# bobocode/lmono

Measured on AMD Instinct MI355X. Metric: KITTI HDL-64 scans/sec (scanRegistration + laserOdometry), higher is better.
Workload: dtype f32 features / f64 solve

## Files before the change

lmono_amd/csrc/batch.hpp:

```cpp
#pragma once
#include "common.hpp"

namespace lmono {

constexpr int kCornerTable = 16384;
constexpr int kSurfTable = 131072;
constexpr unsigned long long kEmptyKey = ~0ull;

struct __attribute__((aligned(16))) GridCell {
    unsigned long long key;
    int start;
    int cnt;
};

struct BatchView {
    const float4 *in;
    const int64_t *off;
    int n_scans;
    int scan0;
    int n_lines;
    int n_limit;
    int has_grid;
    float min_range;
    float4 *cloud;
    float *curv;
    int8_t *label;
    uint8_t *gap;
    int8_t *ring_tmp;
    int *seg_hist;
    int *scan_ends;
    int *scan_half;
    float *scan_ori;
    int *ring_begin;
    int *n_cloud;
    int *status;
    int *sel_sharp;
    int *sel_sharp_n;
    int *sel_flat;
    int *sel_flat_n;
    float4 *lf_tmp;
    int *lf_n;
    int *sel_todo;
    int *li_todo;
    int *vox_todo;
    float4 *sharp;
    float4 *less_sharp;
    float4 *flat;
    float4 *less_flat;
    int *feat_n;
    int *line_first_ge;
    int *line_last_le;
    GridCell *cg_cell;
    GridCell *sg_cell;
    float4 *cg_pts;
    float4 *sg_pts;
    float4 *lbc_pts;
    float4 *lbs_pts;
    int *lb_start;
    float4 *lb_elev;
    int *grid_mask;
};

}
```

lmono_amd/csrc/frontend.hip:

```cpp
#include "batch.hpp"

namespace lmono {

__device__ __forceinline__ int ring_of(float angle, int n_lines, bool &discard)
{
    int id = 0;
    discard = false;
    if (n_lines == 16) {
        id = (int)((double)((angle + 15.0f) / 2.0f) + 0.5);
        if (id > n_lines - 1 || id < 0) discard = true;
    } else if (n_lines == 32) {
        id = (int)(((double)angle + 92.0 / 3.0) * 3.0 / 4.0);
        if (id > n_lines - 1 || id < 0) discard = true;
    } else {
        if ((double)angle >= -8.83)
            id = (int)((double)(2.0f - angle) * 3.0 + 0.5);
        else
            id = n_lines / 2 + (int)((-8.83 - (double)angle) * 2.0 + 0.5);
        if ((double)angle > 2.0 || (double)angle < -24.33 || id > 50 || id < 0) discard = true;
    }
    return id;
}

__device__ __forceinline__ bool point_valid(const float4 &p, float mr2)
// ... 873 lines not shown
        for (int w = 0; w < wave; w++) base += scr[48 + w];
        n_out = scr[48] + scr[49] + scr[50] + scr[51];
        int o = base;
        for (int t = t_lo; t < t_hi; t++) {
            const unsigned int c = (unsigned int)(keys[t] >> 32);
            if (t == 0 || c != (unsigned int)(keys[t - 1] >> 32)) {
                float sx = 0.f, sy = 0.f, sz = 0.f, si = 0.f;
                int cnt = 0;
                for (int u = t; u < nseg && (unsigned int)(keys[u] >> 32) == c; u++) {
                    const int i0 = (int)(keys[u] & 0xffffffffull);
                    int rl = 1;
                    while (i0 + rl < len && ((contw[(i0 + rl) >> 6] >> ((i0 + rl) & 63)) & 1ull)) rl++;
                    for (int b4 = 0; b4 < rl; b4 += 4) {
                        float4 q4[4];
#pragma unroll
                        for (int k = 0; k < 4; k++) q4[k] = b4 + k < rl ? cl[i0 + b4 + k] : make_float4(0.f, 0.f, 0.f, 0.f);
#pragma unroll
                        for (int k = 0; k < 4; k++) if (b4 + k < rl) { sx += q4[k].x; sy += q4[k].y; sz += q4[k].z; si += q4[k].w; }
                    }
                    cnt += rl;
                }
                const float fc = (float)cnt;
                outp[o++] = make_float4(sx / fc, sy / fc, sz / fc, si / fc);
            }
        }
    }
    VT(6)
#ifdef LMONO_VOX_PROF
    if (blockIdx.x == 20 && blockIdx.y == 3 && tid == 0) printf("VOX len %d nseg %d nout %d | load %lld bbox+cell %lld heads %lld sort %lld runs %lld accum %lld\n", len, nseg, n_out, vt[1]-vt[0], vt[2]-vt[1], vt[3]-vt[2], vt[4]-vt[3], vt[5]-vt[4], vt[6]-vt[5]);
#endif
    if (tid == 0) b.lf_n[s * 64 + r] = n_out;
}

#ifndef LMONO_COMPACT_T
#define LMONO_COMPACT_T 256
#endif
constexpr int kCompT = LMONO_COMPACT_T;
static_assert(kCompT >= 256 && kCompT % 64 == 0, "the four prefixes take one wave each");

template <int kT>
__device__ __forceinline__ void compact_scan(const BatchView &b, int s, int &n_ls_out, int &n_lf_out)
{
    const int tid = threadIdx.x;
    const int64_t off = b.off[s];
    constexpr int NE = kMaxRings * kSectors;
    __shared__ int pre_sh[NE + 1], pre_ls[NE + 1], pre_fl[NE + 1], pre_lf[kMaxRings + 1];
    const int *nsh = b.sel_sharp_n + s * NE;
    const int *nfl = b.sel_flat_n + s * NE;
    {
        const int lane = tid & 63, wave = tid >> 6;
        constexpr int kPer = NE / 64;
        int c[kPer], sum = 0;
        if (wave < 4) {
        const int *srcp = wave <= 1 ? nsh : (wave == 2 ? nfl : b.lf_n + s * 64);
#pragma unroll
        for (int q = 0; q < kPer; q++) {
            const int e = lane * kPer + q;
            const bool on = wave < 3 || e < kMaxRings;
            c[q] = srcp[on ? e : 0];
            if (!on) c[q] = 0;
        }
#pragma unroll
        for (int q = 0; q < kPer; q++) {
            if (wave == 0) c[q] = min(c[q], 2);
            sum += c[q];
        }
        const int incl = wave_scan_incl(sum);
        int run = incl - sum;
        int *dst = wave == 0 ? pre_sh : (wave == 1 ? pre_ls : (wave == 2 ? pre_fl : pre_lf));
        const int n_e = wave == 3 ? kMaxRings : NE;
#pragma unroll
        for (int q = 0; q < kPer; q++) {
// ... 74 lines not shown
        for (int q = 0; q < 4; q++) {
            const int j = j0 + kT * q;
            if (j < n_lf) {
                lf[j] = v4[q];
                int v = (int)v4[q].w;
                v = v < 0 ? 0 : (v > 65 ? 65 : v);
                atomicMin(&s_first[1][v], j);
                atomicMax(&s_last[1][v], j);
            }
        }
    }
    if (tid == 0) {
        b.feat_n[s * 4 + 0] = pre_sh[NE]; b.feat_n[s * 4 + 1] = pre_ls[NE];
        b.feat_n[s * 4 + 2] = pre_fl[NE]; b.feat_n[s * 4 + 3] = n_lf;
    }
    __syncthreads();
    for (int x = tid; x < 2 * 66 * 66; x += kT) {
        const int cld = x / (66 * 66), y = x % (66 * 66), a = y / 66, bb = y % 66;
        if (a >= bb + 3 && s_first[cld][a] < s_last[cld][bb]) s_flag[cld] = 1;
    }
    __syncthreads();
    if (tid == 0 || tid == 64) {
        const int cld = tid >> 6;
        const int n = cld ? n_lf : pre_ls[NE];
        int *first_ge = b.line_first_ge + (size_t)(s * 2 + cld) * 66, *last_le = b.line_last_le + (size_t)(s * 2 + cld) * 66;
        int m = n;
        for (int t = 65; t >= 0; t--) { m = min(m, s_first[cld][t] == INT_MAX ? n : s_first[cld][t]); first_ge[t] = m; }
        int M = -1;
        for (int t = 0; t <= 65; t++) { M = max(M, s_last[cld][t]); last_le[t] = M; }
        if (s_flag[cld]) atomicOr(b.status + s, kStatusIrregularLines);
    }
    n_ls_out = pre_ls[NE]; n_lf_out = n_lf;
}

__global__ __launch_bounds__(kCompT) void k_compact(BatchView b)
{
    int n_ls, n_lf;
    compact_scan<kCompT>(b, b.scan0 + blockIdx.x, n_ls, n_lf);
}

}
```

lmono_amd/csrc/lmono_hip.hip:

```cpp
#include "frontend.hip"
#include "odometry.hip"
#include "corr_flat.hip"
#include "mapping.hip"
#include "ba.hip"
#include "ba_solve.hip"
#include "feat.hip"
#include "marg.hip"

#include <string>
#include <vector>
#include <thread>
#include <mutex>
#include <condition_variable>
#include <atomic>
#include <functional>
#include <memory>
#include <chrono>
#include <algorithm>
#include <cstdio>
#include <cstring>

constexpr int kListGrid = 256;

using namespace lmono;
// ... 95 lines not shown
#ifdef LMONO_DIAG_SEARCH
extern "C" const char *lmono_version(void) { return "lmono-hip 0.4 (gfx950, diagnostic build: + hash-grid search)"; }
#else
extern "C" const char *lmono_version(void) { return "lmono-hip 0.4 (gfx950)"; }
#endif

extern "C" lmono_ctx *lmono_create(int device)
{
    int n = 0;
    if (hipGetDeviceCount(&n) != hipSuccess || n <= 0 || device < 0 || device >= n) return nullptr;
    if (hipSetDevice(device) != hipSuccess) return nullptr;
    lmono_ctx *c = new lmono_ctx();
    c->device = device;
    if (const char *e = getenv("LMONO_ODOM_STREAM_PRIORITY")) c->odom_prio = atoi(e) != 0;
    if (const char *e = getenv("GPU_MAX_HW_QUEUES")) c->many_queues = atoi(e) >= 8;
    {
        hipDeviceProp_t prop;
        if (hipGetDeviceProperties(&prop, device) != hipSuccess) { delete c; return nullptr; }
        c->n_cu = prop.multiProcessorCount;
        int per_cu = 0;
        if (hipOccupancyMaxActiveBlocksPerMultiprocessor(&per_cu, (const void *)k_ba_solve<true, false>, kBaT, 0) != hipSuccess || per_cu < 1) per_cu = 1;
        c->cluster_budget = std::max(8, c->n_cu * per_cu / 2);
        c->map_budget = std::max(8, c->n_cu / 2);
        if (const char *e = getenv("LMONO_CLUSTER_BUDGET")) { const int v = atoi(e); if (v >= 1) c->cluster_budget = c->map_budget = v; }
    }
    if (hipMalloc((void **)&c->stats_d, 320) != hipSuccess || hipMemset(c->stats_d, 0, 320) != hipSuccess) { delete c; return nullptr; }
    if (hipFuncSetAttribute((const void *)k_select, hipFuncAttributeMaxDynamicSharedMemorySize, 4 * sel_slice_bytes(kRingCap) + 4 * kSelScratch) != hipSuccess) { delete c; return nullptr; }
    if (hipFuncSetAttribute((const void *)k_voxel<kVoxSmallSlots, kVoxSmallBits, true>, hipFuncAttributeMaxDynamicSharedMemorySize, kVoxLdsSmall) != hipSuccess) { delete c; return nullptr; }
    if (hipFuncSetAttribute((const void *)k_voxel<kVoxBigSlots, kVoxBigBits, false>, hipFuncAttributeMaxDynamicSharedMemorySize, kVoxLdsBig) != hipSuccess) { delete c; return nullptr; }
    if (hipFuncSetAttribute((const void *)k_lm_solve, hipFuncAttributeMaxDynamicSharedMemorySize, kLmRecLds) != hipSuccess) { delete c; return nullptr; }
#ifdef LMONO_DIAG_SEARCH
    if (hipFuncSetAttribute((const void *)k_grid_build, hipFuncAttributeMaxDynamicSharedMemorySize, kGridLds) != hipSuccess) { delete c; return nullptr; }
#endif
    if (hipFuncSetAttribute((const void *)k_line_index<true>, hipFuncAttributeMaxDynamicSharedMemorySize, kLiLdsHalf) != hipSuccess) { delete c; return nullptr; }
    if (hipFuncSetAttribute((const void *)k_compact_index, hipFuncAttributeMaxDynamicSharedMemorySize, kLiLdsHalf) != hipSuccess) { delete c; return nullptr; }
    if (hipFuncSetAttribute((const void *)k_line_index<false>, hipFuncAttributeMaxDynamicSharedMemorySize, kLiLdsFull) != hipSuccess) { delete c; return nullptr; }
    if (hipFuncSetAttribute((const void *)k_marginalize, hipFuncAttributeMaxDynamicSharedMemorySize, (int)sizeof(MargLds)) != hipSuccess) { delete c; return nullptr; }
    if (hipFuncSetAttribute((const void *)k_marg_second_new, hipFuncAttributeMaxDynamicSharedMemorySize, (int)sizeof(Marg2Lds)) != hipSuccess) { delete c; return nullptr; }
#ifdef LMONO_TILE_PROF
    {
        int nb = 0;
        (void)hipOccupancyMaxActiveBlocksPerMultiprocessor(&nb, (const void *)k_corr_flat, kCfT, 0);
        std::fprintf(stderr, "[lmono diag] k_corr_flat: %d workgroups of %d threads per CU by the occupancy query, static LDS %zu B\n", nb, kCfT, sizeof(CfLds));
    }
#endif
    return c;
}

extern "C" void lmono_destroy(lmono_ctx *c)
{
    if (!c) return;
#ifdef LMONO_BOUNDS
    {
        unsigned long long o[4] = { 0, 0, 0, 0 };
        (void)hipDeviceSynchronize();
        if (hipMemcpyFromSymbol(o, HIP_SYMBOL(g_ba_oob), sizeof(o)) == hipSuccess)
            fprintf(stderr, "[lmono bounds] k_ba_solve: %llu access(es) outside the batch's allocation (first: ba_solve.hip:%llu, byte offset %lld, block %llu)\n", o[0], o[1], (long long)o[2], o[3]);
    }
#endif
    for (auto &s : c->sets) { for (auto &e : s.e) (void)hipEventDestroy(e); for (auto &e : s.kev) (void)hipEventDestroy(e); }
    if (c->stats_d) (void)hipFree(c->stats_d);
    for (auto &s : c->gstream) if (s) (void)hipStreamDestroy(s);
    if (c->copy_stream) (void)hipStreamDestroy(c->copy_stream);
    for (void *h : c->stage_all) (void)hipHostFree(h);
    if (c->own_stream) (void)hipStreamDestroy(c->own_stream);
    for (auto &ch : c->arena) (void)hipFree(ch.base);
    for (auto &e : c->gev) if (e) (void)hipEventDestroy(e);
    delete c;
}
// ... 56 lines not shown
    void *q = nullptr;
    if (hipMalloc(&q, (count > 0 ? count : 1) * sizeof(T)) != hipSuccess) return false;
    b->allocs.push_back(q);
    p = (T *)q;
    return true;
}

extern "C" void lmono_batch_destroy(lmono_scan_batch *b)
{
    if (!b) return;
    for (void *p : b->allocs) (void)hipFree(p);
    for (auto &e : b->rep_ev) if (e) (void)hipEventDestroy(e);
    if (b->staged_ev) (void)hipEventDestroy(b->staged_ev);
    if (b->in_free_ev) (void)hipEventDestroy(b->in_free_ev);
    delete b;
}

extern "C" lmono_scan_batch *lmono_batch_create(lmono_ctx *c, int n_cap, int64_t pts_cap)
{
    if (!c || n_cap <= 0 || pts_cap <= 0) return nullptr;
    if (hipSetDevice(c->device) != hipSuccess) return nullptr;
    lmono_scan_batch *b = new lmono_scan_batch();
    b->ctx = c; b->n_cap = n_cap; b->pts_cap = pts_cap;
    BatchView &v = b->v;
    const size_t T = (size_t)pts_cap, N = (size_t)n_cap;
    bool ok = true;
    ok = ok && dalloc(b, b->off_d, N + 1);
    ok = ok && dalloc(b, v.cloud, T) && dalloc(b, v.curv, T) && dalloc(b, v.label, T) && dalloc(b, v.gap, T);
    ok = ok && dalloc(b, v.ring_tmp, T);
    ok = ok && dalloc(b, v.seg_hist, ((T >> 10) + N + 1) * 64) && dalloc(b, v.scan_ends, N * 2) && dalloc(b, v.scan_half, N) && dalloc(b, v.scan_ori, N * 2);
    ok = ok && dalloc(b, v.ring_begin, N * 65) && dalloc(b, v.n_cloud, N) && dalloc(b, v.status, N);
    ok = ok && dalloc(b, v.sel_sharp, N * 64 * 6 * 20) && dalloc(b, v.sel_sharp_n, N * 64 * 6);
    ok = ok && dalloc(b, v.sel_flat, N * 64 * 6 * 4) && dalloc(b, v.sel_flat_n, N * 64 * 6);
    ok = ok && dalloc(b, v.lf_tmp, T) && dalloc(b, v.lf_n, N * 64) && dalloc(b, v.vox_todo, N * 64 + 1) && dalloc(b, v.sel_todo, N * 64 + 1) && dalloc(b, v.li_todo, N * 2 + 1);
    ok = ok && dalloc(b, v.sharp, N * kMaxSharp) && dalloc(b, v.less_sharp, N * kMaxLessSharp);
    ok = ok && dalloc(b, v.flat, N * kMaxFlat) && dalloc(b, v.less_flat, T);
    ok = ok && dalloc(b, v.feat_n, N * 4) && dalloc(b, v.line_first_ge, N * 2 * 66) && dalloc(b, v.line_last_le, N * 2 * 66);
    ok = ok && dalloc(b, v.cg_cell, N * kCornerTable) && dalloc(b, v.sg_cell, N * kSurfTable);
    ok = ok && dalloc(b, v.cg_pts, N * kMaxLessSharp) && dalloc(b, v.sg_pts, T) && dalloc(b, v.grid_mask, N * 2);
    ok = ok && dalloc(b, v.lbc_pts, N * kMaxLessSharp + kLbPad) && dalloc(b, v.lbs_pts, T + kLbPad) && dalloc(b, v.lb_start, N * 2 * (kLineKeys + 1)) && dalloc(b, v.lb_elev, N * 2 * 66);
    ok = ok && dalloc(b, b->incr, N * 7) && dalloc(b, b->poses, N * 7) && dalloc(b, b->xq, 8);
    ok = ok && dalloc(b, b->corr_pair, (size_t)kMaxQueries * 4) && dalloc(b, b->crec_pair, (size_t)kMaxQueries * 4);
    if (!ok) {
        c->err = "lmono_batch_create: hipMalloc failed";
        lmono_batch_destroy(b);
        return nullptr;
    }
    v.off = b->off_d;
    return b;
}

static int rings_used(int n_lines) { return n_lines == 64 ? 51 : n_lines; }

static int check_launch(lmono_ctx *c, const char *what)
{
    hipError_t e = hipGetLastError();
    if (e != hipSuccess) { c->err = std::string(what) + ": " + hipGetErrorString(e); return LMONO_ENODEV; }
    return LMONO_OK;
}

static int scanreg_launch(lmono_ctx *c, lmono_scan_batch *b, int scan0, int n_scans, int64_t max_pts, int n_limit = 0)
{
    BatchView v = b->v;
    v.scan0 = scan0; v.n_limit = n_limit;
    hipStream_t st = c->stream;
    c->ev = c->next_set();
    if (!c->ev) { c->err = "hipEventCreate failed"; return LMONO_ENODEV; }
    c->sets[c->n_sets - 1].reg = true;
    HIP_TRY(c, hipMemsetAsync(v.status + scan0, 0, sizeof(int) * n_scans, st));
    HIP_TRY(c, hipMemsetAsync(v.vox_todo, 0, sizeof(int), st));
    HIP_TRY(c, hipMemsetAsync(v.sel_todo, 0, sizeof(int), st));
    HIP_TRY(c, hipMemsetAsync(v.li_todo, 0, sizeof(int), st));
    HIP_TRY(c, hipEventRecord(c->ev[0], st));
    const int rt_tiles = (int)((max_pts + kRtTile - 1) / kRtTile);
    hipLaunchKernelGGL(k_ring_ends, dim3(n_scans), dim3(256), 0, st, v);
    if (rt_tiles > 0) hipLaunchKernelGGL(k_ring_tag, dim3(rt_tiles, n_scans), dim3(kRtT), 0, st, v);
    hipLaunchKernelGGL(k_ring_offsets, dim3(n_scans), dim3(64), 0, st, v);
    if (rt_tiles > 0) hipLaunchKernelGGL(k_ring_scatter, dim3(rt_tiles, n_scans), dim3(kRtT), 0, st, v);
    HIP_TRY(c, hipEventRecord(c->ev[1], st));
    const int tiles = (int)((max_pts + kCurvTile - 1) / kCurvTile);
#if !LMONO_FUSE_CURV_SELECT
    if (tiles > 0) hipLaunchKernelGGL(k_curvature, dim3(tiles, n_scans), dim3(256), 0, st, v);
#else
    (void)tiles;
#endif
    HIP_TRY(c, hipEventRecord(c->ev[2], st));
    const int n_rings = rings_used(b->v.n_lines);
    HIP_TRY(c, hipMemsetAsync(v.sel_sharp_n + (size_t)scan0 * 64 * 6, 0, sizeof(int) * (size_t)n_scans * 64 * 6, st));
    HIP_TRY(c, hipMemsetAsync(v.sel_flat_n + (size_t)scan0 * 64 * 6, 0, sizeof(int) * (size_t)n_scans * 64 * 6, st));
    HIP_TRY(c, hipMemsetAsync(v.lf_n + (size_t)scan0 * 64, 0, sizeof(int) * (size_t)n_scans * 64, st));
    hipLaunchKernelGGL(k_select, dim3((n_rings + 3) / 4, n_scans), dim3(256), 4 * sel_slice_bytes(kSelSmallCap) + 4 * kSelScratch, st, v, kSelSmallCap, 0);
    hipLaunchKernelGGL(k_select, dim3(kSelBigGrid), dim3(256), 4 * sel_slice_bytes(kRingCap) + 4 * kSelScratch, st, v, (int)kRingCap, 1);
    HIP_TRY(c, hipEventRecord(c->ev[3], st));
    hipLaunchKernelGGL((k_voxel<kVoxSmallSlots, kVoxSmallBits, true>), dim3(n_rings, n_scans), dim3(256), kVoxLdsSmall, st, v);
    hipLaunchKernelGGL((k_voxel<kVoxBigSlots, kVoxBigBits, false>), dim3(kVoxBigGrid), dim3(256), kVoxLdsBig, st, v);
    HIP_TRY(c, hipEventRecord(c->ev[4], st));
#if LMONO_FUSE_COMPACT_INDEX
    hipLaunchKernelGGL(k_compact_index, dim3(n_scans), dim3(kLiT), kLiLdsHalf, st, v);
#else
    hipLaunchKernelGGL(k_compact, dim3(n_scans), dim3(kCompT), 0, st, v);
#endif
    HIP_TRY(c, hipEventRecord(c->ev[5], st));
#ifdef LMONO_DIAG_SEARCH
    if (c->opt[LMONO_OPT_CORR_TILE] != 3) {
        hipLaunchKernelGGL(k_grid_build, dim3(n_scans, 1 + kGridPar), dim3(1024), kGridLds, st, v);
        b->grid_built = true; v.has_grid = 1; b->v.has_grid = 1;
    }
#endif
    HIP_TRY(c, hipEventRecord(c->ev[6], st));
#if !LMONO_FUSE_COMPACT_INDEX
    hipLaunchKernelGGL(k_line_index<true>, dim3(n_scans, 2), dim3(kLiT), kLiLdsHalf, st, v);
#endif
    hipLaunchKernelGGL(k_line_index<false>, dim3(kLiBigGrid), dim3(kLiT), kLiLdsFull, st, v);
    HIP_TRY(c, hipEventRecord(c->ev[7], st));
    return check_launch(c, "scanreg kernels");
}

extern "C" int lmono_scanreg_batch(lmono_ctx *c, lmono_scan_batch *b, const float *xyzi_d, const int64_t *offsets_h,
                                   int n_scans, int n_lines, float min_range);

extern "C" int lmono_scanreg_batch_h(lmono_ctx *c, lmono_scan_batch *b, const float *xyzi_h, const int64_t *offsets_h,
                                     int n_scans, int n_lines, float min_range)
{
    if (!c || !b || !xyzi_h || !offsets_h || n_scans <= 0) return LMONO_EINVAL;
    if (offsets_h[0] != 0) { c->err = "offsets must start at 0"; return LMONO_EINVAL; }
    const int64_t total = offsets_h[n_scans];
    if (total < 0 || total > b->pts_cap) { c->err = "batch: too many points"; return LMONO_ECAPACITY; }
    HIP_TRY(c, hipSetDevice(c->device));
    if (!b->in_owned) {
        void *q = nullptr;
        HIP_TRY(c, hipMalloc(&q, (size_t)(b->pts_cap > 0 ? b->pts_cap : 1) * 16));
        b->allocs.push_back(q);
        b->in_owned = (float *)q;
    }
    if (total > 0) {
        HIP_TRY(c, hipMemcpyAsync(b->in_owned, xyzi_h, (size_t)total * 16, hipMemcpyHostToDevice, c->stream));
        HIP_TRY(c, hipStreamSynchronize(c->stream));
    }
    return lmono_scanreg_batch(c, b, b->in_owned, offsets_h, n_scans, n_lines, min_range);
}

extern "C" int lmono_scanreg_batch(lmono_ctx *c, lmono_scan_batch *b, const float *xyzi_d, const int64_t *offsets_h,
                                   int n_scans, int n_lines, float min_range)
{
    if (!c || !b || !xyzi_d || !offsets_h || n_scans <= 0) return LMONO_EINVAL;
    if (n_lines != 16 && n_lines != 32 && n_lines != 64) { c->err = "n_lines must be 16, 32 or 64"; return LMONO_EINVAL; }
// ... 98 lines not shown
        }
    }
    {
        unsigned long long st[40] = { 0 };
        HIP_TRY(c, hipMemcpy(st, c->stats_d, 320, hipMemcpyDeviceToHost));
        sum[12] = (double)st[0];
        for (int i = 1; i < 40 && 12 + i < cap; i++) ms[12 + i] = (double)st[i];
    }
    for (int i = 0; i < cap && i < 13; i++) ms[i] = sum[i];
    if (n_scanreg_calls) *n_scanreg_calls = nr;
    if (n_odom_calls) *n_odom_calls = no;
    return LMONO_OK;
}

extern "C" int lmono_batch_counts(lmono_ctx *c, lmono_scan_batch *b, int32_t *counts_h)
{
    if (!c || !b || !counts_h || !b->registered) return LMONO_EINVAL;
    const int n = b->n_scans;
    std::vector<int> nc(n), fn(n * 4), stt(n);
    HIP_TRY(c, hipStreamSynchronize(c->stream));
    HIP_TRY(c, hipMemcpy(nc.data(), b->v.n_cloud, sizeof(int) * n, hipMemcpyDeviceToHost));
    HIP_TRY(c, hipMemcpy(fn.data(), b->v.feat_n, sizeof(int) * n * 4, hipMemcpyDeviceToHost));
    HIP_TRY(c, hipMemcpy(stt.data(), b->v.status, sizeof(int) * n, hipMemcpyDeviceToHost));
    for (int s = 0; s < n; s++) {
        counts_h[6 * s] = nc[s];
        for (int k = 0; k < 4; k++) counts_h[6 * s + 1 + k] = fn[4 * s + k];
        counts_h[6 * s + 5] = stt[s];
    }
    return LMONO_OK;
}

extern "C" int lmono_batch_get_cloud(lmono_ctx *c, lmono_scan_batch *b, int scan, int which, float *out_h, int cap)
{
    if (!c || !b || !out_h || !b->registered || scan < 0 || scan >= b->n_scans || which < 0 || which > 4) return LMONO_EINVAL;
    HIP_TRY(c, hipStreamSynchronize(c->stream));
    int n = 0;
    const float4 *src = nullptr;
    int fn[4];
    HIP_TRY(c, hipMemcpy(fn, b->v.feat_n + scan * 4, sizeof(fn), hipMemcpyDeviceToHost));
    switch (which) {
    case 0: HIP_TRY(c, hipMemcpy(&n, b->v.n_cloud + scan, sizeof(int), hipMemcpyDeviceToHost)); src = b->v.cloud + b->off_h[scan]; break;
    case 1: n = fn[0]; src = b->v.sharp + (size_t)scan * kMaxSharp; break;
    case 2: n = fn[1]; src = b->v.less_sharp + (size_t)scan * kMaxLessSharp; break;
    case 3: n = fn[2]; src = b->v.flat + (size_t)scan * kMaxFlat; break;
    default: n = fn[3]; src = b->v.less_flat + b->off_h[scan]; break;
    }
    if (n > cap) { c->err = "get_cloud: output capacity too small"; return LMONO_ECAPACITY; }
    if (n > 0) HIP_TRY(c, hipMemcpy(out_h, src, sizeof(float4) * n, hipMemcpyDeviceToHost));
    return n;
}

extern "C" int lmono_batch_get_curvature(lmono_ctx *c, lmono_scan_batch *b, int scan, float *curv_h, int32_t *label_h, int cap)
{
    if (!c || !b || !b->registered || scan < 0 || scan >= b->n_scans) return LMONO_EINVAL;
    HIP_TRY(c, hipStreamSynchronize(c->stream));
    int n = 0;
    HIP_TRY(c, hipMemcpy(&n, b->v.n_cloud + scan, sizeof(int), hipMemcpyDeviceToHost));
    if (n > cap) { c->err = "get_curvature: output capacity too small"; return LMONO_ECAPACITY; }
    if (curv_h && n > 0) HIP_TRY(c, hipMemcpy(curv_h, b->v.curv + b->off_h[scan], sizeof(float) * n, hipMemcpyDeviceToHost));
    if (label_h && n > 0) {
        std::vector<int8_t> tmp(n);
        HIP_TRY(c, hipMemcpy(tmp.data(), b->v.label + b->off_h[scan], n, hipMemcpyDeviceToHost));
        for (int i = 0; i < n; i++) label_h[i] = tmp[i];
    }
    return n;
}

static int ensure_odom_ws(lmono_ctx *c, lmono_scan_batch *b, int n_chains)
{
    if (n_chains <= b->chains_cap) return LMONO_OK;
    bool ok = dalloc(b, b->state, (size_t)n_chains * 8) && dalloc(b, b->corr, (size_t)n_chains * kMaxQueries * 4) &&
              dalloc(b, b->lm_info, (size_t)n_chains * 4) && dalloc(b, b->crec, (size_t)n_chains * kMaxQueries * 4) &&
              dalloc(b, b->seed, (size_t)n_chains * kMaxQueries) && dalloc(b, b->wl, 8 * ((size_t)n_chains * kMaxQueries + 1)) &&
              dalloc(b, b->ws, (size_t)n_chains * 8) && dalloc(b, b->resid_d, (size_t)n_chains) && dalloc(b, b->rstat, (size_t)n_chains * 4) &&
              dalloc(b, b->rcount, (size_t)n_chains + 2);
    if (!ok) { c->err = "odometry workspace: hipMalloc failed"; return LMONO_ENOMEM; }
    b->chains_cap = n_chains;
    return LMONO_OK;
// ... 2253 lines not shown
```

lmono_amd/csrc/odometry.hip:

```cpp
#include "batch.hpp"

namespace lmono {

constexpr float kCell = 1.0f;
constexpr float kInvCell = 1.0f;
constexpr int kMaxShell = 6;
constexpr int kCoordOff = 1 << 20;
constexpr int kRunMaxCount = 32767;
__device__ __forceinline__ int pack_run(int start, int count) { return start | (count << 17); }

__device__ __forceinline__ unsigned long long cell_key(int cx, int cy, int cz)
{
    return ((unsigned long long)(unsigned int)(cx + kCoordOff) << 42) |
           ((unsigned long long)(unsigned int)(cy + kCoordOff) << 21) |
           (unsigned long long)(unsigned int)(cz + kCoordOff);
}
__device__ __forceinline__ unsigned int hash_key(unsigned long long k)
{
    const unsigned int cz = (unsigned int)(k & 0x1fffffull), cy = (unsigned int)((k >> 21) & 0x1fffffull), cx = (unsigned int)(k >> 42);
    unsigned int h = (cx * 73856093u) ^ (cy * 19349663u) ^ (cz * 83492791u);
    h ^= h >> 15;
    return h;
}

// ... 388 lines not shown
    return r == r ? r : 1e300;
}

constexpr int kAzBins = 384;
constexpr int kLineKeys = 66 * kAzBins;
__device__ __forceinline__ int lb_key(int bin, int line) { return line * kAzBins + bin; }
constexpr int kLbPad = 4;
template <class F>
__device__ __forceinline__ void lb_for_runs(const int *table, int b_lo, int nbins, int va, int vb, F f)
{
    const int b_end = b_lo + nbins;
    for (int part = 0; part < 2; part++) {
        if (part == 1 && b_end <= kAzBins) break;
        const int p0 = part ? 0 : b_lo, p1 = part ? b_end - kAzBins : min(b_end, kAzBins);
        for (int v = va; v <= vb; v++) { const int s0 = table[v * kAzBins + p0]; f(s0, table[v * kAzBins + p1] - s0); }
    }
}

__device__ __forceinline__ int az_bin(float x, float y)
{
    const float t = (atan2f(y, x) + 3.14159265f) * (kAzBins / 6.28318531f);
    const int bi = (int)t;
    return bi < 0 ? 0 : (bi >= kAzBins ? kAzBins - 1 : bi);
}
__device__ __forceinline__ int line_of(float w)
{
    const int v = (int)w;
    return v < 0 ? 0 : (v > 65 ? 65 : v);
}
__device__ __forceinline__ float elev_of(float x, float y, float z) { return atan2f(z, sqrtf(x * x + y * y)); }
__device__ __forceinline__ int f2ord(float f) { const int i = __float_as_int(f); return i >= 0 ? i : i ^ 0x7fffffff; }
__device__ __forceinline__ float ord2f(int i) { return __int_as_float(i >= 0 ? i : i ^ 0x7fffffff); }

constexpr int kLiT = 1024;
constexpr int kLiLdsHalf = kLineKeys * 2, kLiLdsFull = kLineKeys * 4;
constexpr int kLiBigGrid = 64;

template <bool kHalf>
__device__ __forceinline__ void line_index_cloud(const BatchView &b, int s, bool surf, int n, int *s_cnt, int *s_wsum, int *s_emin, int *s_emax)
{
    const int tid = threadIdx.x, lane = tid & 63, wave = tid >> 6;
    const float4 *src = surf ? b.less_flat + b.off[s] : b.less_sharp + (size_t)s * kMaxLessSharp;
    float4 *dst = surf ? b.lbs_pts + b.off[s] : b.lbc_pts + (size_t)s * kMaxLessSharp;
    int *table = b.lb_start + (size_t)(s * 2 + (surf ? 1 : 0)) * (kLineKeys + 1);
    unsigned int *s_c32 = (unsigned int *)s_cnt;
    constexpr int kWords = kHalf ? kLineKeys / 2 : kLineKeys;
    static_assert(kLineKeys % 2 == 0, "two 16-bit counters per LDS word");
    auto bump = [&](int key) -> int {
        if (kHalf) { const int sh = (key & 1) * 16; return (int)((atomicAdd(&s_c32[key >> 1], 1u << sh) >> sh) & 0xffffu); }
        return atomicAdd(&s_cnt[key], 1);
    };
    for (int i = tid; i < kWords; i += kLiT) s_cnt[i] = 0;
    if (tid < 66) { s_emin[tid] = INT_MAX; s_emax[tid] = INT_MIN; }
    __syncthreads();
    for (int base = 0; base < n; base += 4 * kLiT) {
        float4 p[4];
#pragma unroll
        for (int q = 0; q < 4; q++) { const int i = base + tid + kLiT * q; p[q] = src[i < n ? i : 0]; }
#pragma unroll
        for (int q = 0; q < 4; q++) {
            const bool ok = base + tid + kLiT * q < n;
            const int ln = line_of(p[q].w);
            if (ok) (void)bump(lb_key(az_bin(p[q].x, p[q].y), ln));
            const unsigned long long act = __ballot(ok);
            if (act == 0ull) continue;
            const int eo = f2ord(elev_of(p[q].x, p[q].y, p[q].z));
// ... 53 lines not shown
            const int i = i0 + kLiT * q;
            if (i < n) {
                const int ln = line_of(p[q].w);
                const int d = bump(lb_key(az_bin(p[q].x, p[q].y), ln));
                dst[d] = make_float4(p[q].x, p[q].y, p[q].z, __int_as_float((i << 7) | ln));
            }
        }
    }
}

template <bool kHalf>
__global__ __launch_bounds__(kLiT) void k_line_index(BatchView b)
{
    extern __shared__ __align__(16) int s_cnt[];
    __shared__ int s_wsum[kLiT / 64], s_emin[66], s_emax[66];
    if (kHalf) {
        const int s = b.scan0 + blockIdx.x;
        const bool surf = blockIdx.y == 1;
        if (b.feat_n[s * 4 + (surf ? 3 : 1)] > 65535) {
            if (threadIdx.x == 0) b.li_todo[1 + atomicAdd(&b.li_todo[0], 1)] = s * 2 + (surf ? 1 : 0);
            return;
        }
        line_index_cloud<true>(b, s, surf, b.feat_n[s * 4 + (surf ? 3 : 1)], s_cnt, s_wsum, s_emin, s_emax);
    } else {
        const int n_todo = b.li_todo[0];
        for (int k = blockIdx.x; k < n_todo; k += gridDim.x) {
            const int e = b.li_todo[1 + k];
            __syncthreads();
            line_index_cloud<false>(b, e >> 1, (e & 1) != 0, b.feat_n[(e >> 1) * 4 + ((e & 1) ? 3 : 1)], s_cnt, s_wsum, s_emin, s_emax);
        }
    }
}

#ifndef LMONO_FUSE_COMPACT_INDEX
#define LMONO_FUSE_COMPACT_INDEX 1
#endif
__global__ __launch_bounds__(kLiT) void k_compact_index(BatchView b)
{
    extern __shared__ __align__(16) int s_cnt[];
    __shared__ int s_wsum[kLiT / 64], s_emin[66], s_emax[66];
    const int s = b.scan0 + blockIdx.x;
    int n_ls, n_lf;
    compact_scan<kLiT>(b, s, n_ls, n_lf);
    for (int cld = 0; cld < 2; cld++) {
        const int n = cld ? n_lf : n_ls;
        __builtin_amdgcn_fence(__ATOMIC_RELEASE, "workgroup");
        __syncthreads();
        __builtin_amdgcn_fence(__ATOMIC_ACQUIRE, "workgroup");
        if (n > 65535) { if (threadIdx.x == 0) b.li_todo[1 + atomicAdd(&b.li_todo[0], 1)] = s * 2 + cld; continue; }
        line_index_cloud<true>(b, s, cld != 0, n, s_cnt, s_wsum, s_emin, s_emax);
    }
}

constexpr float kArcSlackBins = 0.05f;
#ifndef LMONO_WR_A0
#define LMONO_WR_A0 0.25f
#define LMONO_WR_B0 0.02f
#define LMONO_WR_A1 1.0f
#define LMONO_WR_B1 0.1f
#endif
__device__ __forceinline__ float walk_radius(int pass, float rho)
{
    return pass == 0 ? LMONO_WR_A0 + LMONO_WR_B0 * rho : (pass == 1 ? LMONO_WR_A1 + LMONO_WR_B1 * rho : (pass == 2 ? fminf(5.0f, 1.0f + 0.0045f * rho * rho) : 5.0f));
}

__device__ __forceinline__ float asin_upper(float x) { return x * (1.0f + 0.5708f * x * x); }

typedef unsigned long long WalkBest;
__device__ __forceinline__ void walk_update(WalkBest &bst, float d, unsigned int seq)
{
    const WalkBest k = ((unsigned long long)__float_as_uint(d) << 32) | seq;
    bst = k < bst ? k : bst;
}

constexpr int kGroup = 32;

__device__ __forceinline__ unsigned int group_ballot(bool pred, int gbase)
{
    return (unsigned int)((__ballot(pred) >> gbase) & 0xffffffffull);
}
__device__ __forceinline__ unsigned int group_min_u32(unsigned int v, int gbase)
{
    v = min(v, dpp_mov_u32<0x111, 0xf>(v, ~0u));
// ... 874 lines not shown
```

Before: 120,100.

## Split compact+line-index into prefix, per-ring gather, and per-line sort kernels

The fused per-scan compact_index kernel (one 1024-thread block per scan, with a fallback big-grid pass for large clouds) is replaced by three kernels. One computes the feature prefix sums per scan, one gathers features per ring while accumulating per-line statistics through atomics, and one builds each line's azimuth bucket table and scatters points for each (line, scan, cloud). The aim is to expose far more parallelism than one block per scan and to drop the overflow todo pass. In exchange it adds two kernel launches and global atomic traffic, and the line-sort kernel rereads the whole ring segment set for every line, which is redundant work.

```diff
diff --git a/lmono_amd/csrc/batch.hpp b/lmono_amd/csrc/batch.hpp
--- a/lmono_amd/csrc/batch.hpp
+++ b/lmono_amd/csrc/batch.hpp
@@ -6,6 +6,13 @@
 constexpr int kCornerTable = 16384;
 constexpr int kSurfTable = 131072;
 constexpr unsigned long long kEmptyKey = ~0ull;
+
+#ifndef LMONO_LEGACY_COMPACT_INDEX
+#define LMONO_LEGACY_COMPACT_INDEX 0
+#endif
+constexpr int kFpSh = 0, kFpLs = 385, kFpFl = 770, kFpLf = 1155, kFeatPre = 1220;
+constexpr int kLaCnt = 0, kLaFirst = 1, kLaLast = 2, kLaEmin = 3, kLaEmax = 4, kLaMask = 5, kLineAcc = 8;
+static_assert(kMaxRings <= 64 && kMaxRings * kSectors + 1 <= kFpLs - kFpSh, "ring masks are 64 bits; prefix slots of 384 + 1 entries");
 
 struct __attribute__((aligned(16))) GridCell {
     unsigned long long key;
@@ -41,7 +48,9 @@
     float4 *lf_tmp;
     int *lf_n;
     int *sel_todo;
+#if LMONO_LEGACY_COMPACT_INDEX
     int *li_todo;
+#endif
     int *vox_todo;
     float4 *sharp;
     float4 *less_sharp;
@@ -50,6 +59,8 @@
     int *feat_n;
     int *line_first_ge;
     int *line_last_le;
+    int *feat_pre;
+    int *line_acc;
     GridCell *cg_cell;
     GridCell *sg_cell;
     float4 *cg_pts;
diff --git a/lmono_amd/csrc/frontend.hip b/lmono_amd/csrc/frontend.hip
--- a/lmono_amd/csrc/frontend.hip
+++ b/lmono_amd/csrc/frontend.hip
@@ -929,12 +929,7 @@
     if (tid == 0) b.lf_n[s * 64 + r] = n_out;
 }
 
-#ifndef LMONO_COMPACT_T
-#define LMONO_COMPACT_T 256
-#endif
-constexpr int kCompT = LMONO_COMPACT_T;
-static_assert(kCompT >= 256 && kCompT % 64 == 0, "the four prefixes take one wave each");
-
+#if LMONO_LEGACY_COMPACT_INDEX
 template <int kT>
 __device__ __forceinline__ void compact_scan(const BatchView &b, int s, int &n_ls_out, int &n_lf_out)
 {
@@ -1075,11 +1070,6 @@
     }
     n_ls_out = pre_ls[NE]; n_lf_out = n_lf;
 }
-
-__global__ __launch_bounds__(kCompT) void k_compact(BatchView b)
-{
-    int n_ls, n_lf;
-    compact_scan<kCompT>(b, b.scan0 + blockIdx.x, n_ls, n_lf);
-}
-
-}
+#endif
+
+}
diff --git a/lmono_amd/csrc/lmono_hip.hip b/lmono_amd/csrc/lmono_hip.hip
--- a/lmono_amd/csrc/lmono_hip.hip
+++ b/lmono_amd/csrc/lmono_hip.hip
@@ -151,9 +151,10 @@
 #ifdef LMONO_DIAG_SEARCH
     if (hipFuncSetAttribute((const void *)k_grid_build, hipFuncAttributeMaxDynamicSharedMemorySize, kGridLds) != hipSuccess) { delete c; return nullptr; }
 #endif
-    if (hipFuncSetAttribute((const void *)k_line_index<true>, hipFuncAttributeMaxDynamicSharedMemorySize, kLiLdsHalf) != hipSuccess) { delete c; return nullptr; }
+#if LMONO_LEGACY_COMPACT_INDEX
     if (hipFuncSetAttribute((const void *)k_compact_index, hipFuncAttributeMaxDynamicSharedMemorySize, kLiLdsHalf) != hipSuccess) { delete c; return nullptr; }
     if (hipFuncSetAttribute((const void *)k_line_index<false>, hipFuncAttributeMaxDynamicSharedMemorySize, kLiLdsFull) != hipSuccess) { delete c; return nullptr; }
+#endif
     if (hipFuncSetAttribute((const void *)k_marginalize, hipFuncAttributeMaxDynamicSharedMemorySize, (int)sizeof(MargLds)) != hipSuccess) { delete c; return nullptr; }
     if (hipFuncSetAttribute((const void *)k_marg_second_new, hipFuncAttributeMaxDynamicSharedMemorySize, (int)sizeof(Marg2Lds)) != hipSuccess) { delete c; return nullptr; }
 #ifdef LMONO_TILE_PROF
@@ -276,10 +277,14 @@
     ok = ok && dalloc(b, v.ring_begin, N * 65) && dalloc(b, v.n_cloud, N) && dalloc(b, v.status, N);
     ok = ok && dalloc(b, v.sel_sharp, N * 64 * 6 * 20) && dalloc(b, v.sel_sharp_n, N * 64 * 6);
     ok = ok && dalloc(b, v.sel_flat, N * 64 * 6 * 4) && dalloc(b, v.sel_flat_n, N * 64 * 6);
-    ok = ok && dalloc(b, v.lf_tmp, T) && dalloc(b, v.lf_n, N * 64) && dalloc(b, v.vox_todo, N * 64 + 1) && dalloc(b, v.sel_todo, N * 64 + 1) && dalloc(b, v.li_todo, N * 2 + 1);
+    ok = ok && dalloc(b, v.lf_tmp, T) && dalloc(b, v.lf_n, N * 64) && dalloc(b, v.vox_todo, N * 64 + 1) && dalloc(b, v.sel_todo, N * 64 + 1);
+#if LMONO_LEGACY_COMPACT_INDEX
+    ok = ok && dalloc(b, v.li_todo, N * 2 + 1);
+#endif
     ok = ok && dalloc(b, v.sharp, N * kMaxSharp) && dalloc(b, v.less_sharp, N * kMaxLessSharp);
     ok = ok && dalloc(b, v.flat, N * kMaxFlat) && dalloc(b, v.less_flat, T);
     ok = ok && dalloc(b, v.feat_n, N * 4) && dalloc(b, v.line_first_ge, N * 2 * 66) && dalloc(b, v.line_last_le, N * 2 * 66);
+    ok = ok && dalloc(b, v.feat_pre, N * kFeatPre) && dalloc(b, v.line_acc, N * 2 * 66 * kLineAcc);
     ok = ok && dalloc(b, v.cg_cell, N * kCornerTable) && dalloc(b, v.sg_cell, N * kSurfTable);
     ok = ok && dalloc(b, v.cg_pts, N * kMaxLessSharp) && dalloc(b, v.sg_pts, T) && dalloc(b, v.grid_mask, N * 2);
     ok = ok && dalloc(b, v.lbc_pts, N * kMaxLessSharp + kLbPad) && dalloc(b, v.lbs_pts, T + kLbPad) && dalloc(b, v.lb_start, N * 2 * (kLineKeys + 1)) && dalloc(b, v.lb_elev, N * 2 * 66);
@@ -314,7 +319,9 @@
     HIP_TRY(c, hipMemsetAsync(v.status + scan0, 0, sizeof(int) * n_scans, st));
     HIP_TRY(c, hipMemsetAsync(v.vox_todo, 0, sizeof(int), st));
     HIP_TRY(c, hipMemsetAsync(v.sel_todo, 0, sizeof(int), st));
+#if LMONO_LEGACY_COMPACT_INDEX
     HIP_TRY(c, hipMemsetAsync(v.li_todo, 0, sizeof(int), st));
+#endif
     HIP_TRY(c, hipEventRecord(c->ev[0], st));
     const int rt_tiles = (int)((max_pts + kRtTile - 1) / kRtTile);
     hipLaunchKernelGGL(k_ring_ends, dim3(n_scans), dim3(256), 0, st, v);
@@ -339,10 +346,12 @@
     hipLaunchKernelGGL((k_voxel<kVoxSmallSlots, kVoxSmallBits, true>), dim3(n_rings, n_scans), dim3(256), kVoxLdsSmall, st, v);
     hipLaunchKernelGGL((k_voxel<kVoxBigSlots, kVoxBigBits, false>), dim3(kVoxBigGrid), dim3(256), kVoxLdsBig, st, v);
     HIP_TRY(c, hipEventRecord(c->ev[4], st));
-#if LMONO_FUSE_COMPACT_INDEX
+#if LMONO_LEGACY_COMPACT_INDEX
     hipLaunchKernelGGL(k_compact_index, dim3(n_scans), dim3(kLiT), kLiLdsHalf, st, v);
 #else
-    hipLaunchKernelGGL(k_compact, dim3(n_scans), dim3(kCompT), 0, st, v);
+    hipLaunchKernelGGL(k_feat_prefix, dim3(n_scans), dim3(kFpT), 0, st, v);
+    hipLaunchKernelGGL(k_feat_ring, dim3(n_rings, n_scans), dim3(kFrT), 0, st, v);
+    hipLaunchKernelGGL(k_line_sort, dim3(66, n_scans, 2), dim3(kLsT), 0, st, v);
 #endif
     HIP_TRY(c, hipEventRecord(c->ev[5], st));
 #ifdef LMONO_DIAG_SEARCH
@@ -352,10 +361,9 @@
     }
 #endif
     HIP_TRY(c, hipEventRecord(c->ev[6], st));
-#if !LMONO_FUSE_COMPACT_INDEX
-    hipLaunchKernelGGL(k_line_index<true>, dim3(n_scans, 2), dim3(kLiT), kLiLdsHalf, st, v);
+#if LMONO_LEGACY_COMPACT_INDEX
+    hipLaunchKernelGGL(k_line_index<false>, dim3(kLiBigGrid), dim3(kLiT), kLiLdsFull, st, v);
 #endif
-    hipLaunchKernelGGL(k_line_index<false>, dim3(kLiBigGrid), dim3(kLiT), kLiLdsFull, st, v);
     HIP_TRY(c, hipEventRecord(c->ev[7], st));
     return check_launch(c, "scanreg kernels");
 }
@@ -520,7 +528,7 @@
 
 extern "C" int lmono_batch_get_cloud(lmono_ctx *c, lmono_scan_batch *b, int scan, int which, float *out_h, int cap)
 {
-    if (!c || !b || !out_h || !b->registered || scan < 0 || scan >= b->n_scans || which < 0 || which > 4) return LMONO_EINVAL;
+    if (!c || !b || !out_h || !b->registered || scan < 0 || scan >= b->n_scans || which < 0 || which > 7) return LMONO_EINVAL;
     HIP_TRY(c, hipStreamSynchronize(c->stream));
     int n = 0;
     const float4 *src = nullptr;
@@ -531,7 +539,21 @@
     case 1: n = fn[0]; src = b->v.sharp + (size_t)scan * kMaxSharp; break;
     case 2: n = fn[1]; src = b->v.less_sharp + (size_t)scan * kMaxLessSharp; break;
     case 3: n = fn[2]; src = b->v.flat + (size_t)scan * kMaxFlat; break;
-    default: n = fn[3]; src = b->v.less_flat + b->off_h[scan]; break;
+    case 4: n = fn[3]; src = b->v.less_flat + b->off_h[scan]; break;
+    case 5: n = fn[1]; src = b->v.lbc_pts + (size_t)scan * kMaxLessSharp; break;
+    case 6: n = fn[3]; src = b->v.lbs_pts + b->off_h[scan]; break;
+    default: {
+        constexpr size_t kTab = 2 * (size_t)(kLineKeys + 1), kWords = kTab + 2 * 66 * 2 + 2 * 66 * 4;
+        n = (int)((kWords + 3) / 4);
+        if (n > cap) { c->err = "get_cloud: output capacity too small"; return LMONO_ECAPACITY; }
+        std::vector<int> w((size_t)n * 4, 0);
+        HIP_TRY(c, hipMemcpy(w.data(), b->v.lb_start + (size_t)scan * kTab, sizeof(int) * kTab, hipMemcpyDeviceToHost));
+        HIP_TRY(c, hipMemcpy(w.data() + kTab, b->v.line_first_ge + (size_t)scan * 2 * 66, sizeof(int) * 2 * 66, hipMemcpyDeviceToHost));
+        HIP_TRY(c, hipMemcpy(w.data() + kTab + 2 * 66, b->v.line_last_le + (size_t)scan * 2 * 66, sizeof(int) * 2 * 66, hipMemcpyDeviceToHost));
+        HIP_TRY(c, hipMemcpy(w.data() + kTab + 4 * 66, b->v.lb_elev + (size_t)scan * 2 * 66, sizeof(float4) * 2 * 66, hipMemcpyDeviceToHost));
+        std::memcpy(out_h, w.data(), sizeof(int) * w.size());
+        return n;
+    }
     }
     if (n > cap) { c->err = "get_cloud: output capacity too small"; return LMONO_ECAPACITY; }
     if (n > 0) HIP_TRY(c, hipMemcpy(out_h, src, sizeof(float4) * n, hipMemcpyDeviceToHost));
diff --git a/lmono_amd/csrc/odometry.hip b/lmono_amd/csrc/odometry.hip
--- a/lmono_amd/csrc/odometry.hip
+++ b/lmono_amd/csrc/odometry.hip
@@ -444,6 +444,7 @@
 __device__ __forceinline__ int f2ord(float f) { const int i = __float_as_int(f); return i >= 0 ? i : i ^ 0x7fffffff; }
 __device__ __forceinline__ float ord2f(int i) { return __int_as_float(i >= 0 ? i : i ^ 0x7fffffff); }
 
+#if LMONO_LEGACY_COMPACT_INDEX
 constexpr int kLiT = 1024;
 constexpr int kLiLdsHalf = kLineKeys * 2, kLiLdsFull = kLineKeys * 4;
 constexpr int kLiBigGrid = 64;
@@ -563,9 +564,6 @@
     }
 }
 
-#ifndef LMONO_FUSE_COMPACT_INDEX
-#define LMONO_FUSE_COMPACT_INDEX 1
-#endif
 __global__ __launch_bounds__(kLiT) void k_compact_index(BatchView b)
 {
     extern __shared__ __align__(16) int s_cnt[];
@@ -580,6 +578,236 @@
         __builtin_amdgcn_fence(__ATOMIC_ACQUIRE, "workgroup");
         if (n > 65535) { if (threadIdx.x == 0) b.li_todo[1 + atomicAdd(&b.li_todo[0], 1)] = s * 2 + cld; continue; }
         line_index_cloud<true>(b, s, cld != 0, n, s_cnt, s_wsum, s_emin, s_emax);
+    }
+}
+#endif
+
+constexpr int kFpT = 256;
+constexpr int kFrT = 256;
+constexpr int kLsT = 256;
+static_assert(kAzBins <= 2 * kLsT, "k_line_sort's prefix takes two bins per thread");
+
+__global__ __launch_bounds__(kFpT) void k_feat_prefix(BatchView b)
+{
+    const int s = b.scan0 + blockIdx.x, tid = threadIdx.x, lane = tid & 63, wave = tid >> 6;
+    constexpr int NE = kMaxRings * kSectors;
+    constexpr int kPer = NE / 64;
+    int *pre = b.feat_pre + (size_t)s * kFeatPre;
+    const int *srcp = wave <= 1 ? b.sel_sharp_n + (size_t)s * NE : (wave == 2 ? b.sel_flat_n + (size_t)s * NE : b.lf_n + (size_t)s * 64);
+    const int n_e = wave == 3 ? kMaxRings : NE;
+    int c[kPer], sum = 0;
+#pragma unroll
+    for (int q = 0; q < kPer; q++) {
+        const int e = lane * kPer + q;
+        c[q] = srcp[e < n_e ? e : 0];
+        if (e >= n_e) c[q] = 0;
+        if (wave == 0) c[q] = min(c[q], 2);
+        sum += c[q];
+    }
+    const int incl = wave_scan_incl(sum);
+    int run = incl - sum;
+    int *dst = pre + (wave == 0 ? kFpSh : (wave == 1 ? kFpLs : (wave == 2 ? kFpFl : kFpLf)));
+#pragma unroll
+    for (int q = 0; q < kPer; q++) {
+        const int e = lane * kPer + q;
+        if (e < n_e) dst[e] = run;
+        run += c[q];
+    }
+    if (lane == 63) { dst[n_e] = run; b.feat_n[s * 4 + wave] = run; }
+    for (int x = tid; x < 2 * 66; x += kFpT) {
+        int *a = b.line_acc + ((size_t)s * 2 * 66 + x) * kLineAcc;
+        a[kLaCnt] = 0; a[kLaFirst] = INT_MAX; a[kLaLast] = -1; a[kLaEmin] = INT_MAX; a[kLaEmax] = INT_MIN; a[kLaMask] = 0; a[kLaMask + 1] = 0;
+    }
+}
+
+__device__ __forceinline__ void line_acc_point(int (*acc)[5], bool ok, const float4 &p, int pos)
+{
+    const unsigned long long act = __ballot(ok);
+    if (act == 0ull) return;
+    const int ln = line_of(p.w);
+    const int eo = f2ord(elev_of(p.x, p.y, p.z));
+    const int ln0 = __shfl(ln, __ffsll((long long)act) - 1);
+    if (__ballot(ok && ln != ln0) == 0ull) {
+        const unsigned int plo = wave_min_u32_uniform(ok ? (unsigned int)pos : ~0u), phi = wave_max_u32_uniform(ok ? (unsigned int)pos : 0u);
+        const unsigned int elo = wave_min_u32_uniform(ok ? (unsigned int)eo ^ 0x80000000u : ~0u);
+        const unsigned int ehi = wave_max_u32_uniform(ok ? (unsigned int)eo ^ 0x80000000u : 0u);
+        if ((threadIdx.x & 63) == 0) {
+            atomicAdd(&acc[ln0][0], __popcll(act));
+            atomicMin(&acc[ln0][1], (int)plo); atomicMax(&acc[ln0][2], (int)phi);
+            atomicMin(&acc[ln0][3], (int)(elo ^ 0x80000000u)); atomicMax(&acc[ln0][4], (int)(ehi ^ 0x80000000u));
+        }
+    } else if (ok) {
+        atomicAdd(&acc[ln][0], 1);
+        atomicMin(&acc[ln][1], pos); atomicMax(&acc[ln][2], pos);
+        atomicMin(&acc[ln][3], eo); atomicMax(&acc[ln][4], eo);
+    }
+}
+
+__global__ __launch_bounds__(kFrT) void k_feat_ring(BatchView b)
+{
+    const int r = blockIdx.x, s = b.scan0 + blockIdx.y, tid = threadIdx.x;
+    constexpr int NE = kMaxRings * kSectors;
+    const int *pre = b.feat_pre + (size_t)s * kFeatPre;
+    __shared__ int s_acc[2][66][5];
+    __shared__ int s_pre[3][kSectors + 1], s_lf[2];
+    if (tid < 2 * 66) {
+        int *a = s_acc[tid / 66][tid % 66];
+        a[0] = 0; a[1] = INT_MAX; a[2] = -1; a[3] = INT_MAX; a[4] = INT_MIN;
+    }
+    if (tid >= 192 && tid < 192 + 3 * (kSectors + 1)) {
+        const int k = tid - 192, w = k / (kSectors + 1), q = k % (kSectors + 1);
+        s_pre[w][q] = pre[(w == 0 ? kFpSh : (w == 1 ? kFpLs : kFpFl)) + r * kSectors + q];
+    }
+    if (tid >= 160 && tid < 162) s_lf[tid - 160] = pre[kFpLf + r + tid - 160];
+    __syncthreads();
+    const int64_t off = b.off[s];
+    const float4 *cl = b.cloud + off;
+    {
+        bool ok = false;
+        int pos = 0;
+        float4 p = make_float4(0.f, 0.f, 0.f, 0.f);
+        if (tid < kSectors * 20) {
+            const int q = tid / 20, k = tid % 20;
+            if (k < s_pre[1][q + 1] - s_pre[1][q]) {
+                ok = true;
+                pos = s_pre[1][q] + k;
+                p = cl[b.sel_sharp[((size_t)s * NE + r * kSectors + q) * 20 + k]];
+                b.less_sharp[(size_t)s * kMaxLessSharp + pos] = p;
+                if (k < 2) b.sharp[(size_t)s * kMaxSharp + s_pre[0][q] + k] = p;
+            }
+        } else if (tid >= 128 && tid < 128 + kSectors * 4) {
+            const int q = (tid - 128) / 4, k = (tid - 128) % 4;
+            if (k < s_pre[2][q + 1] - s_pre[2][q])
+                b.flat[(size_t)s * kMaxFlat + s_pre[2][q] + k] = cl[b.sel_flat[((size_t)s * NE + r * kSectors + q) * 4 + k]];
+        }
+        line_acc_point(s_acc[0], ok, p, pos);
+    }
+    const int lf0 = s_lf[0], nr = s_lf[1] - lf0;
+    const float4 *src = b.lf_tmp + off + b.ring_begin[s * 65 + r];
+    float4 *dst = b.less_flat + off + lf0;
+    for (int i0 = 0; i0 < nr; i0 += 4 * kFrT) {
+        float4 p[4];
+#pragma unroll
+        for (int q = 0; q < 4; q++) { const int i = i0 + tid + kFrT * q; p[q] = src[i < nr ? i : 0]; }
+#pragma unroll
+        for (int q = 0; q < 4; q++) {
+            const int i = i0 + tid + kFrT * q;
+            if (i < nr) dst[i] = p[q];
+            line_acc_point(s_acc[1], i < nr, p[q], lf0 + i);
+        }
+    }
+    __syncthreads();
+    if (tid < 2 * 66) {
+        const int cld = tid / 66, v = tid % 66;
+        const int *a = s_acc[cld][v];
+        if (a[0] > 0) {
+            int *g = b.line_acc + ((size_t)(s * 2 + cld) * 66 + v) * kLineAcc;
+            atomicAdd(&g[kLaCnt], a[0]);
+            atomicMin(&g[kLaFirst], a[1]); atomicMax(&g[kLaLast], a[2]);
+            atomicMin(&g[kLaEmin], a[3]); atomicMax(&g[kLaEmax], a[4]);
+            atomicOr(&g[kLaMask + (r >> 5)], 1 << (r & 31));
+        }
+    }
+}
+
+__global__ __launch_bounds__(kLsT) void k_line_sort(BatchView b)
+{
+    const int ln = blockIdx.x, s = b.scan0 + blockIdx.y, cld = blockIdx.z, tid = threadIdx.x, lane = tid & 63, wave = tid >> 6;
+    const int *acc = b.line_acc + (size_t)(s * 2 + cld) * 66 * kLineAcc;
+    const int *pre = b.feat_pre + (size_t)s * kFeatPre;
+    const int n = b.feat_n[s * 4 + (cld ? 3 : 1)];
+    int *table = b.lb_start + (size_t)(s * 2 + cld) * (kLineKeys + 1);
+    __shared__ int s_cnt[kAzBins];
+    __shared__ int s_lcnt[66], s_wsum[kLsT / 64], s_seg[kMaxRings][2], s_nseg, s_tot;
+    if (tid < 66) s_lcnt[tid] = acc[tid * kLineAcc + kLaCnt];
+    for (int i = tid; i < kAzBins; i += kLsT) s_cnt[i] = 0;
+    if (wave == 0) {
+        const unsigned long long m = (unsigned long long)(unsigned int)acc[ln * kLineAcc + kLaMask]
+                                   | ((unsigned long long)(unsigned int)acc[ln * kLineAcc + kLaMask + 1] << 32);
+        const bool on = lane < kMaxRings && ((m >> lane) & 1ull);
+        int a = 0, len = 0;
+        if (on) {
+            a = cld ? pre[kFpLf + lane] : pre[kFpLs + lane * kSectors];
+            len = (cld ? pre[kFpLf + lane + 1] : pre[kFpLs + (lane + 1) * kSectors]) - a;
+        }
+        const int incl = wave_scan_incl(len);
+        const int k = __popcll(m & ((1ull << lane) - 1ull));
+        if (on) { s_seg[k][0] = a; s_seg[k][1] = incl - len; }
+        if (lane == 63) { s_nseg = __popcll(m); s_tot = incl; }
+    }
+    __syncthreads();
+    int line_base = 0;
+    for (int v = 0; v < ln; v++) line_base += s_lcnt[v];
+    if (ln == 0) {
+        __shared__ int s_first[66], s_last[66], s_emin[66], s_emax[66], s_flag;
+        if (tid < 66) {
+            const int *a = acc + tid * kLineAcc;
+            s_first[tid] = a[kLaFirst]; s_last[tid] = a[kLaLast]; s_emin[tid] = a[kLaEmin]; s_emax[tid] = a[kLaEmax];
+        }
+        if (tid == 0) s_flag = 0;
+        __syncthreads();
+        for (int x = tid; x < 66 * 66; x += kLsT) {
+            const int a = x / 66, bb = x % 66;
+            if (a >= bb + 3 && s_first[a] < s_last[bb]) s_flag = 1;
+        }
+        if (tid < 66) {
+            float4 *el = b.lb_elev + (size_t)(s * 2 + cld) * 66;
+            float A = 1e30f, B = -1e30f;
+            for (int v = 0; v <= tid; v++) if (s_emin[v] != INT_MAX) A = fminf(A, ord2f(s_emin[v]));
+            for (int v = tid; v < 66; v++) if (s_emin[v] != INT_MAX) B = fmaxf(B, ord2f(s_emax[v]));
+            el[tid] = s_emin[tid] == INT_MAX ? make_float4(1e30f, -1e30f, A, B) : make_float4(ord2f(s_emin[tid]), ord2f(s_emax[tid]), A, B);
+        }
+        if (tid == 64) table[kLineKeys] = n;
+        __syncthreads();
+        if (tid == 0) {
+            int *first_ge = b.line_first_ge + (size_t)(s * 2 + cld) * 66, *last_le = b.line_last_le + (size_t)(s * 2 + cld) * 66;
+            int mm = n;
+            for (int t = 65; t >= 0; t--) { mm = min(mm, s_first[t] == INT_MAX ? n : s_first[t]); first_ge[t] = mm; }
+            int M = -1;
+            for (int t = 0; t <= 65; t++) { M = max(M, s_last[t]); last_le[t] = M; }
+            if (s_flag) atomicOr(b.status + s, kStatusIrregularLines);
+        }
+    }
+    const float4 *src = cld ? b.less_flat + b.off[s] : b.less_sharp + (size_t)s * kMaxLessSharp;
+    float4 *dst = cld ? b.lbs_pts + b.off[s] : b.lbc_pts + (size_t)s * kMaxLessSharp;
+    const int tot = s_tot, nseg = s_nseg;
+    auto at = [&](int j) -> int {
+        int k = 0;
+        while (k + 1 < nseg && s_seg[k + 1][1] <= j) k++;
+        return s_seg[k][0] + (j - s_seg[k][1]);
+    };
+    for (int j0 = tid; j0 < tot; j0 += 4 * kLsT) {
+        float4 p[4];
+#pragma unroll
+        for (int q = 0; q < 4; q++) { const int j = j0 + kLsT * q; p[q] = src[j < tot ? at(j) : 0]; }
+#pragma unroll
+        for (int q = 0; q < 4; q++)
+            if (j0 + kLsT * q < tot && line_of(p[q].w) == ln) atomicAdd(&s_cnt[az_bin(p[q].x, p[q].y)], 1);
+    }
+    __syncthreads();
+    {
+        const int c0 = 2 * tid < kAzBins ? s_cnt[2 * tid] : 0, c1 = 2 * tid + 1 < kAzBins ? s_cnt[2 * tid + 1] : 0;
+        const int loc = c0 + c1, incl = wave_scan_incl(loc);
+        if (lane == 63) s_wsum[wave] = incl;
+        __syncthreads();
+        int run = line_base + incl - loc;
+        for (int w = 0; w < wave; w++) run += s_wsum[w];
+        if (2 * tid < kAzBins) { table[ln * kAzBins + 2 * tid] = run; s_cnt[2 * tid] = run; }
+        if (2 * tid + 1 < kAzBins) { table[ln * kAzBins + 2 * tid + 1] = run + c0; s_cnt[2 * tid + 1] = run + c0; }
+    }
+    __syncthreads();
+    for (int j0 = tid; j0 < tot; j0 += 4 * kLsT) {
+        float4 p[4];
+        int idx[4];
+#pragma unroll
+        for (int q = 0; q < 4; q++) { const int j = j0 + kLsT * q; idx[q] = j < tot ? at(j) : 0; p[q] = src[idx[q]]; }
+#pragma unroll
+        for (int q = 0; q < 4; q++) {
+            if (j0 + kLsT * q < tot && line_of(p[q].w) == ln) {
+                const int d = atomicAdd(&s_cnt[az_bin(p[q].x, p[q].y)], 1);
+                dst[d] = make_float4(p[q].x, p[q].y, p[q].z, __int_as_float((idx[q] << 7) | ln));
+            }
+        }
     }
 }
 
```

New measurement: 120,300, median of 5. About the same (+0.1%).
